# ruizhecao96/CMGAN

Measured on NVIDIA H100. Metric: utterances/sec (2 s @16 kHz) generator fwd+bwd, higher is better.
Workload: dtype tf32

## Files before the change

### cmgan_b200/csrc/gemm_tc.cu

```cuda
#include <cuda.h>

#include "common.cuh"
#include "../../include/cmgan_b200.h"
#include "gemm_device.cuh"
#include "tc_ptx.cuh"

namespace {
using namespace cmgan_gemm;
using namespace cmgan_tc;

constexpr int BM = 64;
constexpr int KC = 32;
constexpr int A_STAGE_BYTES = BM * KC * 4;
constexpr int NPROD = 128;
constexpr int NTHREADS = 256;
constexpr int SLAB = 64;
constexpr int STG_LD = SLAB + 4;
constexpr int STG_BYTES = 4 * 16 * STG_LD * 4;
constexpr int SMEM_LIMIT = 227 * 1024;
constexpr int SMEM_LIMIT2 = 112 * 1024;
constexpr int RESIDENT_MAX = 96 * 1024;

__global__ void pack_b_kernel(const float* __restrict__ B, long sb_tap, long sb_k, long sb_n, int Cin, int ntaps, int N, int BN,
                              float* __restrict__ out) {
    long total = (long)ntaps * (Cin / KC) * BN * KC;
    long i = (long)blockIdx.x * blockDim.x + threadIdx.x;
    if (i >= total) return;
    int kk = (int)(i % KC); long t = i / KC; int n = (int)(t % BN); long chunk = t / BN;
    int cpt = Cin / KC;
    int tap = (int)(chunk / cpt), kc = (int)(chunk % cpt);
    float v = 0.f;
    if (n < N) v = to_tf32(__ldg(B + (long)tap * sb_tap + (long)(kc * KC + kk) * sb_k + (long)n * sb_n));
    int c = kk >> 2, j = kk & 3;
    out[(chunk * BN + n) * KC + ((c ^ (n & 7)) << 2) + j] = v;
}

__global__ void pack_all_kernel(const CmganPackDesc* __restrict__ descs) {
    const CmganPackDesc d = descs[blockIdx.y];
    const int Cin = (int)d.Cin, N = (int)d.N;
    const long total = d.ntaps * (Cin / KC) * (long)N * KC;
    for (long i = (long)blockIdx.x * blockDim.x + threadIdx.x; i < total; i += (long)gridDim.x * blockDim.x) {
        int kk = (int)(i % KC); long t = i / KC; int n = (int)(t % N); long chunk = t / N;
        int cpt = Cin / KC;
        int tap = (int)(chunk / cpt), kc = (int)(chunk % cpt);
        float v = to_tf32(__ldg(d.src + (long)tap * d.sb_tap + (long)(kc * KC + kk) * d.sb_k + (long)n * d.sb_n));
        int c = kk >> 2, j = kk & 3;
        d.dst[(chunk * N + n) * KC + ((c ^ (n & 7)) << 2) + j] = v;
    }
}

struct TcCfg { int BN, stages, resident, ntiles, tma, nfx, nty, W, H; };
constexpr int PW = 8, PH = 8;

template <bool ASYNC_A, int NBMAX, int EPI, bool PATCH>
__global__ void __launch_bounds__(NTHREADS, NBMAX == 4 ? 2 : 1) gemm_rows_tc_kernel(const __grid_constant__ CmganGemmArgs g, const float* __restrict__ Bp,
                                                                                  const TcCfg cfg, const __grid_constant__ CUtensorMap tmA) {
    extern __shared__ uint8_t smem_raw[];
    const uint32_t base = (smem_u32(smem_raw) + 1023u) & ~1023u;
    uint8_t* base_ptr = smem_raw + (base - smem_u32(smem_raw));
    const int BN = cfg.BN, stages = cfg.stages;
    const int b_tile_bytes = BN * KC * 4;
    const int cpt = g.Cin / KC;
    const int nchunks = cpt * g.ntaps;
    const uint32_t sA = base;
    const uint32_t sB = sA + stages * A_STAGE_BYTES;
    const uint32_t b_region = (uint32_t)(cfg.resident ? nchunks : stages) * b_tile_bytes;
    const uint32_t sStg = sB + b_region;
    const uint32_t bars = sStg + STG_BYTES;
    auto full_bar = [&](int s) { return bars + 8u * s; };
    auto empty_bar = [&](int s) { return bars + 8u * (stages + s); };
    const uint32_t bready_bar = bars + 8u * (2 * stages);

    const int tid = threadIdx.x, warp = tid >> 5, lane = tid & 31;
    const int ntiles = cfg.ntiles;
    const int my_tiles = (ntiles - (int)blockIdx.x + (int)gridDim.x - 1) / (int)gridDim.x;

    if (tid == 0) {
        for (int s = 0; s < stages; ++s) { mbar_init(full_bar(s), cfg.tma ? 1 : NPROD + (cfg.resident ? 0 : 1)); mbar_init(empty_bar(s), 4); }
        mbar_init(bready_bar, 1);
        fence_barrier_init();
    }
    __syncthreads();

    if (warp < 4) {
        const int c = tid & 7;
        const int rr = tid >> 3;
        uint32_t dst_off[4];
#pragma unroll
        for (int i = 0; i < 4; ++i) { const int r = rr + 16 * i; dst_off[i] = r * 128 + ((c ^ (r & 7)) << 4); }
        const long total = (long)my_tiles * nchunks;
        if (tid == 0 && cfg.resident) {
            mbar_arrive_expect_tx(bready_bar, (uint32_t)(nchunks * b_tile_bytes));
            for (int ch = 0; ch < nchunks; ++ch)
                bulk_g2s(sB + ch * b_tile_bytes, Bp + (long)ch * BN * KC, (uint32_t)b_tile_bytes, bready_bar);
        }
#define B_STAGE(q, s)                                                                                                    \
        if (tid == 0 && !cfg.resident) {                                                                                 \
            if (!cfg.tma) mbar_arrive_expect_tx(full_bar(s), (uint32_t)b_tile_bytes);                                    \
            bulk_g2s(sB + (s) * b_tile_bytes, Bp + (long)((q) % nchunks) * BN * KC, (uint32_t)b_tile_bytes, full_bar(s)); \
        }

        if (ASYNC_A && cfg.tma) {
            if (tid == 0) {
                for (long q = 0; q < total; ++q) {
                    const int lt = (int)(q / nchunks), ch = (int)(q - (long)lt * nchunks);
                    const int s = (int)(q % stages);
                    const uint32_t par = (uint32_t)((q / stages) & 1);
                    mbar_wait(empty_bar(s), par ^ 1u);
                    mbar_arrive_expect_tx(full_bar(s), (uint32_t)(A_STAGE_BYTES + (cfg.resident ? 0 : b_tile_bytes)));
                    B_STAGE(q, s)
                    const int tile = blockIdx.x + lt * gridDim.x;
                    if (!PATCH) {
                        tma_load_2d(sA + s * A_STAGE_BYTES, &tmA, ch * KC, tile * BM, full_bar(s));
                    } else {
                        const int fx = tile % cfg.nfx, ty = (tile / cfg.nfx) % cfg.nty, bimg = tile / (cfg.nfx * cfg.nty);
                        const int tap = ch / cpt, kc = ch - tap * cpt;
                        tma_load_4d(sA + s * A_STAGE_BYTES, &tmA, kc * KC, fx * PW + g.dx[tap], ty * PH + g.dy[tap], bimg, full_bar(s));
                    }
                }
            }
            __syncwarp();
        } else if (ASYNC_A) {
            const int LAG = stages >= 3 ? 2 : 1;
            long rowoff[4];
            RowInfo ri[4];
            int cur_tile = -1, cur_tap = -1;
            for (long q = 0; q < total + LAG; ++q) {
                if (q < total) {
                    const int lt = (int)(q / nchunks), ch = (int)(q - (long)lt * nchunks);
                    const int s = (int)(q % stages);
                    const uint32_t par = (uint32_t)((q / stages) & 1);
                    const int tap = ch / cpt, k0 = (ch - tap * cpt) * KC + c * 4;
                    if (lt != cur_tile) {
                        cur_tile = lt; cur_tap = -1;
                        const int m0 = (blockIdx.x + lt * gridDim.x) * BM;
#pragma unroll
                        for (int i = 0; i < 4; ++i) ri[i] = decode_row(g, m0 + rr + 16 * i);
                    }
                    if (tap != cur_tap) {
                        cur_tap = tap;
#pragma unroll
                        for (int i = 0; i < 4; ++i) {
                            long r = in_row_of(g, ri[i], tap);
                            rowoff[i] = r < 0 ? -1 : g.tap_off[tap] + r * g.lda;
                        }
                    }
                    mbar_wait(empty_bar(s), par ^ 1u);
                    B_STAGE(q, s)
                    const uint32_t sbase = sA + s * A_STAGE_BYTES;
#pragma unroll
                    for (int i = 0; i < 4; ++i) {
                        const bool ok = rowoff[i] >= 0;
                        cp_async16(sbase + dst_off[i], g.A + (ok ? rowoff[i] + k0 : 0), ok ? 16u : 0u);
                    }
                }
                cp_async_commit();
                const long done = q - LAG;
                if (done >= 0) {
                    if (LAG == 2) cp_async_wait<2>(); else cp_async_wait<1>();
                    fence_proxy_async();
                    mbar_arrive(full_bar((int)(done % stages)));
                }
            }
        } else {
            float mean[4], rstd[4];
            RowInfo ri[4];
            int cur_tile = -1;
            for (long q = 0; q < total; ++q) {
                const int lt = (int)(q / nchunks), ch = (int)(q - (long)lt * nchunks);
                const int s = (int)(q % stages);
                const uint32_t par = (uint32_t)((q / stages) & 1);
                const int tap = ch / cpt, k0 = (ch - tap * cpt) * KC + c * 4;
                if (lt != cur_tile) {
                    cur_tile = lt;
                    const int m0 = (blockIdx.x + lt * gridDim.x) * BM;
#pragma unroll
                    for (int i = 0; i < 4; ++i) {
                        ri[i] = decode_row(g, m0 + rr + 16 * i);
                        mean[i] = 0.f; rstd[i] = 1.f;
                        if (g.pro == CMGAN_PRO_LN) {
                            long r = in_row_of(g, ri[i], 0);
                            if (r >= 0) { float2 st = __ldg(reinterpret_cast<const float2*>(g.p0) + r); mean[i] = st.x; rstd[i] = st.y; }
                        }
                    }
                }
                ChunkParams cp;
                load_chunk_params(g, k0, cp);
                float4 v[4];
                long rows[4];
#pragma unroll
                for (int i = 0; i < 4; ++i) {
                    rows[i] = in_row_of(g, ri[i], tap);
                    v[i] = rows[i] >= 0 ? __ldg(reinterpret_cast<const float4*>(g.A + g.tap_off[tap] + rows[i] * g.lda + k0)) : make_float4(0.f, 0.f, 0.f, 0.f);
                }
#pragma unroll
                for (int i = 0; i < 4; ++i)
                    if (rows[i] >= 0) v[i] = transform4(g, v[i], rows[i], k0, mean[i], rstd[i], cp);
                mbar_wait(empty_bar(s), par ^ 1u);
                B_STAGE(q, s)
                const uint32_t sbase = sA + s * A_STAGE_BYTES;
#pragma unroll
                for (int i = 0; i < 4; ++i)
                    asm volatile("st.shared.v4.f32 [%0], {%1, %2, %3, %4};" ::"r"(sbase + dst_off[i]), "f"(to_tf32(v[i].x)), "f"(to_tf32(v[i].y)),
                                 "f"(to_tf32(v[i].z)), "f"(to_tf32(v[i].w)) : "memory");
                fence_proxy_async();
                mbar_arrive(full_bar(s));
            }
        }
#undef B_STAGE
    } else {
        const int cw = warp - 4;
        const int nb = BN / 16;
        float acc[NBMAX][8];
#pragma unroll
        for (int j = 0; j < NBMAX; ++j)
#pragma unroll
            for (int i = 0; i < 8; ++i) acc[j][i] = 0.f;
        float* stg = reinterpret_cast<float*>(base_ptr + (sStg - base)) + cw * 16 * STG_LD;
        const int col4 = (lane & 15) * 4;
        const int rsub = lane >> 4;
        const int fg = lane >> 2, ft = lane & 3;
        constexpr bool DROPS = EPI == CMGAN_EPI_DROP_RES || EPI == CMGAN_EPI_DSWISH_DROP || EPI == CMGAN_EPI_SWISH_DUAL;
        const uint32_t seed32 = DROPS ? cmgan_seed32(eff_seed(g)) : 0u;
        const uint32_t thr16 = g.drop_thr >> 16;
        const bool drop_on = DROPS && g.drop_thr != 0u;
        constexpr bool patch = PATCH;
        const float inv_keep = g.inv_keep, alpha = g.alpha;
        const float* xbase = nullptr;
        long ldx = 0;
        if (EPI == CMGAN_EPI_DROP_RES) { xbase = g.R; ldx = g.ldr; }
        else if (EPI == CMGAN_EPI_DSWISH_DROP || EPI == CMGAN_EPI_DBNSWISH) { xbase = g.aux; ldx = g.ldaux; }
        else if (EPI == CMGAN_EPI_ACC) { xbase = g.C; ldx = g.ldc; }
        if (cfg.resident) mbar_wait(bready_bar, 0);
        long q = 0;
        for (int lt = 0; lt < my_tiles; ++lt) {
            for (int ch = 0; ch < nchunks; ++ch, ++q) {
                const int s = (int)(q % stages);
                const uint32_t par = (uint32_t)((q / stages) & 1);
                mbar_wait(full_bar(s), par);
                const uint64_t adesc = gmma_desc_sw128(sA + s * A_STAGE_BYTES);
                const uint64_t bdesc = gmma_desc_sw128(sB + (cfg.resident ? ch : s) * b_tile_bytes);
                wgmma_fence();
                mma_chunk_n<NBMAX>(nb, acc, adesc, bdesc, ch == 0);
                wgmma_commit();
                wgmma_wait<0>();
                __syncwarp();
                if (lane == 0) mbar_arrive(empty_bar(s));
            }
            const int tile = blockIdx.x + lt * gridDim.x;
            long mfirst;
            int hi_rows, vhi, vlo;
            if (patch) {
                const int fx = tile % cfg.nfx, ty = (tile / cfg.nfx) % cfg.nty, bimg = tile / (cfg.nfx * cfg.nty);
                const int y0 = ty * PH + cw * 2, x0 = fx * PW;
                mfirst = ((long)bimg * cfg.H + y0) * cfg.W + x0 + rsub;
                hi_rows = cfg.W; vhi = cfg.H - y0; vlo = cfg.W - x0;
            } else {
                const int mrow0 = tile * BM + cw * 16;
                mfirst = (long)mrow0 + rsub;
                hi_rows = 8; vhi = 2; vlo = g.M - mrow0;
            }
            auto row_ok = [&](int ps) { return patch ? ((ps >> 2) < vhi && 2 * (ps & 3) + rsub < vlo) : (2 * ps + rsub < vlo); };
            auto row_delta = [&](int ps) { return (long)(ps >> 2) * hi_rows + 2 * (ps & 3); };
            const bool any_row = row_ok(0);
#pragma unroll
            for (int sl = 0; sl < NBMAX / 4; ++sl) {
                const int n0 = sl * SLAB;
                if (n0 >= BN) break;
                const int ncols = min(SLAB, BN - n0);
#pragma unroll
                for (int jj = 0; jj < 4; ++jj) {
                    if (16 * jj >= ncols) break;
                    const float* d = acc[4 * sl + jj];
#pragma unroll
                    for (int i = 0; i < 2; ++i) {
                        const int col = 16 * jj + 8 * i + 2 * ft;
                        *reinterpret_cast<float2*>(stg + fg * STG_LD + col) = make_float2(d[4 * i], d[4 * i + 1]);
                        *reinterpret_cast<float2*>(stg + (fg + 8) * STG_LD + col) = make_float2(d[4 * i + 2], d[4 * i + 3]);
                    }
                }
                __syncwarp();
                if (col4 < ncols && any_row) {
                    const int n = n0 + col4;
                    float4 bias4 = make_float4(0.f, 0.f, 0.f, 0.f), e0v = bias4, e1v = bias4;
                    if (g.bias) bias4 = __ldg(reinterpret_cast<const float4*>(g.bias + n));
                    if (EPI == CMGAN_EPI_DBNSWISH) { e0v = __ldg(reinterpret_cast<const float4*>(g.e0 + n)); e1v = __ldg(reinterpret_cast<const float4*>(g.e1 + n)); }
                    float* cptr = g.C ? g.C + mfirst * g.ldc + n : nullptr;
                    float* c2ptr = EPI == CMGAN_EPI_SWISH_DUAL ? g.C2 + mfirst * g.ldc2 + n : nullptr;
                    const float* xp = xbase ? xbase + mfirst * ldx + n : nullptr;
                    const float* sptr = stg + rsub * STG_LD + col4;
                    const long ldc = g.ldc, ldc2 = g.ldc2;
                    const uint32_t pair = (uint32_t)(((unsigned long long)mfirst * (unsigned long long)g.N + (unsigned long long)n) >> 1);
                    const uint32_t phalf = (uint32_t)g.N >> 1;
#pragma unroll
                    for (int b4 = 0; b4 < 2; ++b4) {
                        float4 ex[4];
#pragma unroll
                        for (int u = 0; u < 4; ++u)
                            ex[u] = (xp && row_ok(b4 * 4 + u)) ? __ldg(reinterpret_cast<const float4*>(xp + row_delta(b4 * 4 + u) * ldx))
                                                                : make_float4(0.f, 0.f, 0.f, 0.f);
#pragma unroll
                        for (int u = 0; u < 4; ++u) {
                            const int ps = b4 * 4 + u;
                            if (!row_ok(ps)) continue;
                            const long rd = row_delta(ps);
                            const float4 a = *reinterpret_cast<const float4*>(sptr + ps * 2 * STG_LD);
                            float v[4] = {a.x + bias4.x, a.y + bias4.y, a.z + bias4.z, a.w + bias4.w};
                            float ds[4] = {1.f, 1.f, 1.f, 1.f};
                            if (DROPS && drop_on) {
                                const uint32_t pr = pair + (uint32_t)rd * phalf;
                                const uint32_t h0 = cmgan_mix32((pr * 0x9E3779B1u) ^ seed32), h1 = cmgan_mix32(((pr + 1u) * 0x9E3779B1u) ^ seed32);
                                ds[0] = (h0 & 0xFFFFu) >= thr16 ? inv_keep : 0.f; ds[1] = (h0 >> 16) >= thr16 ? inv_keep : 0.f;
                                ds[2] = (h1 & 0xFFFFu) >= thr16 ? inv_keep : 0.f; ds[3] = (h1 >> 16) >= thr16 ? inv_keep : 0.f;
                            }
                            const float x[4] = {ex[u].x, ex[u].y, ex[u].z, ex[u].w};
                            if (EPI == CMGAN_EPI_SWISH_DUAL) {
                                if (cptr) *reinterpret_cast<float4*>(cptr + rd * ldc) = make_float4(v[0], v[1], v[2], v[3]);
#pragma unroll
                                for (int j = 0; j < 4; ++j) v[j] = to_tf32(swishf_(v[j]) * ds[j]);
                                *reinterpret_cast<float4*>(c2ptr + rd * ldc2) = make_float4(v[0], v[1], v[2], v[3]);
                                continue;
                            }
                            if (EPI == CMGAN_EPI_DROP_RES) {
#pragma unroll
                                for (int j = 0; j < 4; ++j) v[j] = alpha * v[j] * ds[j] + (xbase ? x[j] : 0.f);
                            } else if (EPI == CMGAN_EPI_DSWISH_DROP) {
#pragma unroll
                                for (int j = 0; j < 4; ++j) v[j] = to_tf32(v[j] * dswishf_(x[j]) * ds[j]);
                            } else if (EPI == CMGAN_EPI_DBNSWISH) {
                                const float sa[4] = {e0v.x, e0v.y, e0v.z, e0v.w}, sb[4] = {e1v.x, e1v.y, e1v.z, e1v.w};
#pragma unroll
                                for (int j = 0; j < 4; ++j) v[j] = v[j] * dswishf_(fmaf(x[j], sa[j], sb[j]));
                            } else if (EPI == CMGAN_EPI_ACC) {
#pragma unroll
                                for (int j = 0; j < 4; ++j) v[j] = alpha * v[j] + x[j];
                            }
                            *reinterpret_cast<float4*>(cptr + rd * ldc) = make_float4(v[0], v[1], v[2], v[3]);
                        }
                    }
                }
                __syncwarp();
            }
        }
    }
}

int tc_supported(const CmganGemmArgs* a) {
    if (a->N % 16 || a->N < 16 || a->N > 256) return 0;
    if (a->Cin % KC) return 0;
    if (a->lda % 4 || ((uintptr_t)a->A & 15)) return 0;
    if (a->C && (a->ldc % 4 || ((uintptr_t)a->C & 15))) return 0;
    if (a->epi == CMGAN_EPI_SWISH_DUAL && (a->ldc2 % 4 || ((uintptr_t)a->C2 & 15))) return 0;
    if (a->bias && ((uintptr_t)a->bias & 15)) return 0;
    for (int t = 0; t < a->ntaps; ++t)
        if (a->tap_off[t] % 4) return 0;
    if (!a->ws || a->ws_floats < (long long)a->N * a->Cin * a->ntaps) return 0;
    if ((uintptr_t)a->ws & 127) return 0;
    if (a->pro == CMGAN_PRO_LN && (((uintptr_t)a->p1 & 15) || ((uintptr_t)a->p2 & 15) || a->ntaps != 1)) return 0;
    if (a->pro == CMGAN_PRO_BN_SWISH && (((uintptr_t)a->p0 & 15) || ((uintptr_t)a->p1 & 15))) return 0;
    if (a->pro == CMGAN_PRO_IN_PRELU && (((uintptr_t)a->p0 & 15) || ((uintptr_t)a->p1 & 15) || ((uintptr_t)a->p2 & 15) || a->pstride % 4)) return 0;
    return 1;
}

int g_num_sms = 0;

using PFN_encodeTiled = CUresult (*)(CUtensorMap*, CUtensorMapDataType, cuuint32_t, void*, const cuuint64_t*, const cuuint64_t*, const cuuint32_t*,
                                      const cuuint32_t*, CUtensorMapInterleave, CUtensorMapSwizzle, CUtensorMapL2promotion, CUtensorMapFloatOOBfill);
PFN_encodeTiled get_encoder() {
    static PFN_encodeTiled encode = nullptr;
    static bool tried = false;
    if (!tried) {
        tried = true;
        void* fn = nullptr;
        cudaDriverEntryPointQueryResult qres;
        if (cudaGetDriverEntryPoint("cuTensorMapEncodeTiled", &fn, cudaEnableDefault, &qres) == cudaSuccess && qres == cudaDriverEntryPointSuccess)
            encode = reinterpret_cast<PFN_encodeTiled>(fn);
    }
    return encode;
}

template <bool ASYNC_A, int NBMAX, int EPI, bool PATCH = false>
int launch_variant(const CmganGemmArgs& a, const TcCfg& cfg, int grid, size_t smem, cudaStream_t st, const CUtensorMap& tm) {
    static bool attr_set = false;
    if (!attr_set) {
        cudaError_t e = cudaFuncSetAttribute(gemm_rows_tc_kernel<ASYNC_A, NBMAX, EPI, PATCH>, cudaFuncAttributeMaxDynamicSharedMemorySize, SMEM_LIMIT);
        if (e != cudaSuccess) { cmgan_set_error("gemm_rows_tc: cudaFuncSetAttribute: %s", cudaGetErrorString(e)); return -1; }
        attr_set = true;
    }
    gemm_rows_tc_kernel<ASYNC_A, NBMAX, EPI, PATCH><<<grid, NTHREADS, smem, st>>>(a, a.ws, cfg, tm);
    return 0;
}

}

int cmgan_gemm_rows_tc_launch(const CmganGemmArgs* a, cudaStream_t st) {
    if (!tc_supported(a)) return 1;
    TcCfg cfg;
    cfg.BN = a->N;
    const int b_tile = cfg.BN * KC * 4;
    const int nchunks = (a->Cin / KC) * a->ntaps;
    cfg.resident = (long)nchunks * b_tile <= RESIDENT_MAX ? 1 : 0;
    const int resident_bytes = cfg.resident ? nchunks * b_tile : 0;
    const int per_stage = A_STAGE_BYTES + (cfg.resident ? 0 : b_tile);
    const int fixed = 1024  + STG_BYTES + 256  + resident_bytes;
    const int ctas = (a->pro == CMGAN_PRO_NONE && cfg.BN <= 64 && fixed + 3 * per_stage <= SMEM_LIMIT2) ? 2 : 1;
    const bool narrow = ctas == 2;
    cfg.stages = ((ctas == 2 ? SMEM_LIMIT2 : SMEM_LIMIT) - fixed) / per_stage;
    if (cfg.stages > 8) cfg.stages = 8;
    if (cfg.stages < 2) return 1;
    cfg.ntiles = cdiv(a->M, BM);
    const size_t smem = (size_t)fixed + (size_t)cfg.stages * per_stage;
    if (g_num_sms == 0) {
        int dev = 0;
        cudaGetDevice(&dev);
        cudaDeviceGetAttribute(&g_num_sms, cudaDevAttrMultiProcessorCount, dev);
    }
    alignas(64) CUtensorMap tm;
    memset(&tm, 0, sizeof(tm));
    cfg.tma = 0;
    cfg.nfx = cfg.nty = 1; cfg.W = cfg.H = 0;
    if (a->pro == CMGAN_PRO_NONE && !a->conv && a->ntaps == 1 && a->lda % 4 == 0) {
        PFN_encodeTiled encode = get_encoder();
        if (encode) {
            const cuuint64_t gdim[2] = {(cuuint64_t)a->Cin, (cuuint64_t)a->M};
            const cuuint64_t gstride[1] = {(cuuint64_t)a->lda * sizeof(float)};
            const cuuint32_t box[2] = {(cuuint32_t)KC, (cuuint32_t)BM};
            const cuuint32_t estr[2] = {1, 1};
            CUresult r = encode(&tm, CU_TENSOR_MAP_DATA_TYPE_FLOAT32, 2, const_cast<float*>(a->A + a->tap_off[0]), gdim, gstride, box, estr,
                                CU_TENSOR_MAP_INTERLEAVE_NONE, CU_TENSOR_MAP_SWIZZLE_128B, CU_TENSOR_MAP_L2_PROMOTION_L2_256B,
                                CU_TENSOR_MAP_FLOAT_OOB_FILL_NONE);
            if (r == CUDA_SUCCESS) cfg.tma = 1;
        }
    }
    bool same_off = true;
    for (int t = 1; t < a->ntaps; ++t) same_off = same_off && a->tap_off[t] == a->tap_off[0];
    if (a->pro == CMGAN_PRO_NONE && (a->epi == CMGAN_EPI_NONE || a->epi == CMGAN_EPI_ACC) && a->conv && a->mul_y == 1 && a->mul_x == 1 && a->div_y == 1 && a->div_x == 1 && a->OH == a->IH &&
        a->OW == a->IW && same_off && a->M % ((long long)a->OH * a->OW) == 0) {
        PFN_encodeTiled encode = get_encoder();
        if (encode) {
            const long long Bn = a->M / ((long long)a->OH * a->OW);
            const cuuint64_t gdim[4] = {(cuuint64_t)a->Cin, (cuuint64_t)a->IW, (cuuint64_t)a->IH, (cuuint64_t)Bn};
            const cuuint64_t gstride[3] = {(cuuint64_t)a->lda * sizeof(float), (cuuint64_t)a->IW * a->lda * sizeof(float),
                                           (cuuint64_t)a->IH * a->IW * a->lda * sizeof(float)};
            const cuuint32_t box[4] = {(cuuint32_t)KC, (cuuint32_t)PW, (cuuint32_t)PH, 1};
            const cuuint32_t estr[4] = {1, 1, 1, 1};
            CUresult r = encode(&tm, CU_TENSOR_MAP_DATA_TYPE_FLOAT32, 4, const_cast<float*>(a->A + a->tap_off[0]), gdim, gstride, box, estr,
                                CU_TENSOR_MAP_INTERLEAVE_NONE, CU_TENSOR_MAP_SWIZZLE_128B, CU_TENSOR_MAP_L2_PROMOTION_L2_256B,
                                CU_TENSOR_MAP_FLOAT_OOB_FILL_NONE);
            const long long nfx = cdiv(a->OW, PW), nty = cdiv(a->OH, PH);
            if (r == CUDA_SUCCESS && Bn * nfx * nty < (1ll << 30)) {
                cfg.tma = 2; cfg.nfx = (int)nfx; cfg.nty = (int)nty; cfg.W = a->OW; cfg.H = a->OH;
                cfg.ntiles = (int)(Bn * nfx * nty);
            }
        }
    }
    if (!a->b_packed) {
        long total = (long)nchunks * cfg.BN * KC;
        pack_b_kernel<<<cdiv(total, 256), 256, 0, st>>>(a->B, a->sb_tap, a->sb_k, a->sb_n, a->Cin, a->ntaps, a->N, cfg.BN, a->ws);
        if (cmgan_check_launch("pack_b_kernel")) return -1;
    }
    const int grid = cfg.ntiles < ctas * g_num_sms ? cfg.ntiles : ctas * g_num_sms;
    const int variant = a->pro != CMGAN_PRO_NONE ? 0 : (narrow ? 1 : 2);
    int rc = -2;
#define CMGAN_TC_LAUNCH(E)                                                                                            \
    case E:                                                                                                           \
        rc = variant == 0   ? launch_variant<false, 16, E>(*a, cfg, grid, smem, st, tm)                               \
             : variant == 1 ? launch_variant<true, 4, E>(*a, cfg, grid, smem, st, tm)                                 \
                            : launch_variant<true, 16, E>(*a, cfg, grid, smem, st, tm);                               \
        break;
    if (cfg.tma == 2) {
        if (a->epi == CMGAN_EPI_NONE)
            rc = narrow ? launch_variant<true, 4, CMGAN_EPI_NONE, true>(*a, cfg, grid, smem, st, tm)
                        : launch_variant<true, 16, CMGAN_EPI_NONE, true>(*a, cfg, grid, smem, st, tm);
        else
            rc = narrow ? launch_variant<true, 4, CMGAN_EPI_ACC, true>(*a, cfg, grid, smem, st, tm)
                        : launch_variant<true, 16, CMGAN_EPI_ACC, true>(*a, cfg, grid, smem, st, tm);
    } else
    switch (a->epi) {
        CMGAN_TC_LAUNCH(CMGAN_EPI_NONE)
        CMGAN_TC_LAUNCH(CMGAN_EPI_DROP_RES)
        CMGAN_TC_LAUNCH(CMGAN_EPI_DSWISH_DROP)
        CMGAN_TC_LAUNCH(CMGAN_EPI_DBNSWISH)
        CMGAN_TC_LAUNCH(CMGAN_EPI_ACC)
        CMGAN_TC_LAUNCH(CMGAN_EPI_SWISH_DUAL)
        default: break;
    }
#undef CMGAN_TC_LAUNCH
    if (rc == -2) { cmgan_set_error("gemm_rows_tc: unknown epilogue %d", a->epi); return -1; }
    if (rc) return -1;
    return cmgan_check_launch("gemm_rows_tc_kernel");
}

CMGAN_API int cmgan_pack_weight(const float* src, float* dst, long long sb_tap, long long sb_k, long long sb_n, int Cin, int ntaps, int N, void* stream) {
    CMGAN_REQUIRE(src && dst && Cin > 0 && Cin % KC == 0 && ntaps >= 1 && N > 0, "cmgan_pack_weight: bad arguments (Cin must be a multiple of %d)", KC);
    const long total = (long)ntaps * Cin * N;
    pack_b_kernel<<<cdiv(total, 256), 256, 0, (cudaStream_t)stream>>>(src, sb_tap, sb_k, sb_n, Cin, ntaps, N, N, dst);
    return cmgan_check_launch("pack_b_kernel");
}

CMGAN_API int cmgan_pack_weights(const CmganPackDesc* descs, int n, void* stream) {
    CMGAN_REQUIRE(descs || n == 0, "cmgan_pack_weights: null table");
    if (n == 0) return 0;
    pack_all_kernel<<<dim3(48, n), 256, 0, (cudaStream_t)stream>>>(descs);
    return cmgan_check_launch("pack_all_kernel");
}
```

### cmgan_b200/csrc/tc_ptx.cuh

```cuda
#pragma once
#include "common.cuh"

namespace cmgan_tc {

__device__ __forceinline__ uint32_t smem_u32(const void* p) { return (uint32_t)__cvta_generic_to_shared(p); }

__device__ __forceinline__ void mbar_init(uint32_t bar, uint32_t count) {
    asm volatile("mbarrier.init.shared::cta.b64 [%0], %1;" ::"r"(bar), "r"(count) : "memory");
}
__device__ __forceinline__ void mbar_arrive(uint32_t bar) {
    asm volatile("mbarrier.arrive.shared::cta.b64 _, [%0];" ::"r"(bar) : "memory");
}
__device__ __forceinline__ void mbar_arrive_expect_tx(uint32_t bar, uint32_t bytes) {
    asm volatile("mbarrier.arrive.expect_tx.shared::cta.b64 _, [%0], %1;" ::"r"(bar), "r"(bytes) : "memory");
}
__device__ __forceinline__ void mbar_wait(uint32_t bar, uint32_t parity) {
    uint32_t done = 0;
    for (uint32_t spin = 0; !done; ++spin) {
        asm volatile("{\n\t.reg .pred p;\n\tmbarrier.try_wait.parity.shared::cta.b64 p, [%1], %2;\n\tselp.u32 %0, 1, 0, p;\n\t}"
                     : "=r"(done) : "r"(bar), "r"(parity) : "memory");
        if (spin > (1u << 28)) __trap();
    }
}
__device__ __forceinline__ bool mbar_test(uint32_t bar, uint32_t parity) {
    uint32_t done;
    asm volatile("{\n\t.reg .pred p;\n\tmbarrier.test_wait.parity.shared::cta.b64 p, [%1], %2;\n\tselp.u32 %0, 1, 0, p;\n\t}"
                 : "=r"(done) : "r"(bar), "r"(parity) : "memory");
    return done != 0;
}
__device__ __forceinline__ void fence_barrier_init() { asm volatile("fence.mbarrier_init.release.cluster;" ::: "memory"); }
__device__ __forceinline__ void fence_proxy_async() { asm volatile("fence.proxy.async.shared::cta;" ::: "memory"); }

__device__ __forceinline__ void bulk_g2s(uint32_t dst_smem, const void* src, uint32_t bytes, uint32_t bar) {
    asm volatile("cp.async.bulk.shared::cluster.global.mbarrier::complete_tx::bytes [%0], [%1], %2, [%3];"
                 ::"r"(dst_smem), "l"(src), "r"(bytes), "r"(bar) : "memory");
}
__device__ __forceinline__ void tma_load_2d(uint32_t dst_smem, const void* tmap, int c0, int c1, uint32_t bar) {
    asm volatile("cp.async.bulk.tensor.2d.shared::cluster.global.mbarrier::complete_tx::bytes [%0], [%1, {%2, %3}], [%4];"
                 ::"r"(dst_smem), "l"(tmap), "r"(c0), "r"(c1), "r"(bar) : "memory");
}
__device__ __forceinline__ void tma_load_3d(uint32_t dst_smem, const void* tmap, int c0, int c1, int c2, uint32_t bar) {
    asm volatile("cp.async.bulk.tensor.3d.shared::cluster.global.mbarrier::complete_tx::bytes [%0], [%1, {%2, %3, %4}], [%5];"
                 ::"r"(dst_smem), "l"(tmap), "r"(c0), "r"(c1), "r"(c2), "r"(bar) : "memory");
}
__device__ __forceinline__ void tma_load_4d(uint32_t dst_smem, const void* tmap, int c0, int c1, int c2, int c3, uint32_t bar) {
    asm volatile("cp.async.bulk.tensor.4d.shared::cluster.global.mbarrier::complete_tx::bytes [%0], [%1, {%2, %3, %4, %5}], [%6];"
                 ::"r"(dst_smem), "l"(tmap), "r"(c0), "r"(c1), "r"(c2), "r"(c3), "r"(bar) : "memory");
}
__device__ __forceinline__ void cp_async16(uint32_t dst_smem, const void* src, uint32_t src_bytes) {
    asm volatile("cp.async.cg.shared.global [%0], [%1], 16, %2;" ::"r"(dst_smem), "l"(src), "r"(src_bytes) : "memory");
}
__device__ __forceinline__ void cp_async8(uint32_t dst_smem, const void* src) {
    asm volatile("cp.async.ca.shared.global [%0], [%1], 8;" ::"r"(dst_smem), "l"(src) : "memory");
}
__device__ __forceinline__ void cp_async_commit() { asm volatile("cp.async.commit_group;" ::: "memory"); }
template <int N>
__device__ __forceinline__ void cp_async_wait() { asm volatile("cp.async.wait_group %0;" ::"n"(N) : "memory"); }

__device__ __forceinline__ float to_tf32(float x) {
    uint32_t r;
    asm("cvt.rna.tf32.f32 %0, %1;" : "=r"(r) : "f"(x));
    return __uint_as_float(r);
}

__device__ __forceinline__ uint64_t gmma_desc_sw128(uint32_t saddr) {
    uint64_t d = 0;
    d |= (uint64_t)((saddr & 0x3FFFF) >> 4);
    d |= (uint64_t)1 << 16;
    d |= (uint64_t)(1024 >> 4) << 32;
    d |= (uint64_t)1 << 62;
    return d;
}
__device__ __forceinline__ void wgmma_fence() { asm volatile("wgmma.fence.sync.aligned;" ::: "memory"); }
__device__ __forceinline__ void wgmma_commit() { asm volatile("wgmma.commit_group.sync.aligned;" ::: "memory"); }
template <int N>
__device__ __forceinline__ void wgmma_wait() { asm volatile("wgmma.wait_group.sync.aligned %0;" ::"n"(N) : "memory"); }
__device__ __forceinline__ void wgmma_m64n16k8_tf32(float d[8], uint64_t adesc, uint64_t bdesc, uint32_t accumulate) {
    asm volatile("{\n\t.reg .pred p;\n\tsetp.ne.b32 p, %10, 0;\n\t"
                 "wgmma.mma_async.sync.aligned.m64n16k8.f32.tf32.tf32 {%0, %1, %2, %3, %4, %5, %6, %7}, %8, %9, p, 1, 1;\n\t}"
                 : "+f"(d[0]), "+f"(d[1]), "+f"(d[2]), "+f"(d[3]), "+f"(d[4]), "+f"(d[5]), "+f"(d[6]), "+f"(d[7])
                 : "l"(adesc), "l"(bdesc), "r"(accumulate));
}
#define CMGAN_D8(b) "+f"(d[b][0]), "+f"(d[b][1]), "+f"(d[b][2]), "+f"(d[b][3]), "+f"(d[b][4]), "+f"(d[b][5]), "+f"(d[b][6]), "+f"(d[b][7])
__device__ __forceinline__ void wgmma_m64n64k8_tf32(float (&d)[4][8], uint64_t adesc, uint64_t bdesc, uint32_t accumulate) {
    asm volatile("{\n\t.reg .pred p;\n\tsetp.ne.b32 p, %34, 0;\n\t"
                 "wgmma.mma_async.sync.aligned.m64n64k8.f32.tf32.tf32 "
                 "{%0, %1, %2, %3, %4, %5, %6, %7, %8, %9, %10, %11, %12, %13, %14, %15, "
                 "%16, %17, %18, %19, %20, %21, %22, %23, %24, %25, %26, %27, %28, %29, %30, %31}, %32, %33, p, 1, 1;\n\t}"
                 : CMGAN_D8(0), CMGAN_D8(1), CMGAN_D8(2), CMGAN_D8(3)
                 : "l"(adesc), "l"(bdesc), "r"(accumulate));
}
__device__ __forceinline__ void wgmma_m64n64k8_tf32_rs(float (&d)[4][8], const uint32_t (&a)[4], uint64_t bdesc, uint32_t accumulate) {
    asm volatile("{\n\t.reg .pred p;\n\tsetp.ne.b32 p, %37, 0;\n\t"
                 "wgmma.mma_async.sync.aligned.m64n64k8.f32.tf32.tf32 "
                 "{%0, %1, %2, %3, %4, %5, %6, %7, %8, %9, %10, %11, %12, %13, %14, %15, "
                 "%16, %17, %18, %19, %20, %21, %22, %23, %24, %25, %26, %27, %28, %29, %30, %31}, {%32, %33, %34, %35}, %36, p, 1, 1;\n\t}"
                 : CMGAN_D8(0), CMGAN_D8(1), CMGAN_D8(2), CMGAN_D8(3)
                 : "r"(a[0]), "r"(a[1]), "r"(a[2]), "r"(a[3]), "l"(bdesc), "r"(accumulate));
}
#undef CMGAN_D8

template <int NB, int NBMAX>
__device__ __forceinline__ void mma_chunk(float (&acc)[NBMAX][8], uint64_t adesc, uint64_t bdesc, bool first) {
#pragma unroll
    for (int k = 0; k < 4; ++k)
#pragma unroll
        for (int j = 0; j < NB; ++j)
            wgmma_m64n16k8_tf32(acc[j], adesc + (uint64_t)(2 * k), bdesc + (uint64_t)(128 * j + 2 * k), (first && k == 0) ? 0u : 1u);
}
template <int NBMAX, int I = 1>
__device__ __forceinline__ void mma_chunk_n(int nb, float (&acc)[NBMAX][8], uint64_t adesc, uint64_t bdesc, bool first) {
    if constexpr (I <= NBMAX) {
        if (nb == I) mma_chunk<I, NBMAX>(acc, adesc, bdesc, first);
        else mma_chunk_n<NBMAX, I + 1>(nb, acc, adesc, bdesc, first);
    }
}

}
```

Before: 90.98.

## Use wide wgmma instructions and overlap MMA with the next chunk's barrier wait

Replaces the per-16-column m64n16k8 wgmma loop with a single wide m64nNk8 instruction (N = 64/128/192/256) per k-step, rounding the column-block count up to a multiple of four. The consumer loop now keeps one wgmma group in flight (wait<1>) and releases the previous stage's buffer late, so tensor-core work overlaps the next stage's barrier wait. It also reduces the producer lag for three-stage rings and adds a host-side early return for non-TMA configurations with fewer than three stages. Rounding up the width may compute wasted columns, and the new early return could reject configurations that used to run.

```diff
diff --git a/cmgan_b200/csrc/gemm_tc.cu b/cmgan_b200/csrc/gemm_tc.cu
--- a/cmgan_b200/csrc/gemm_tc.cu
+++ b/cmgan_b200/csrc/gemm_tc.cu
@@ -51,6 +51,38 @@
 
 struct TcCfg { int BN, stages, resident, ntiles, tma, nfx, nty, W, H; };
 constexpr int PW = 8, PH = 8;
+
+struct TileRing { uint32_t sA, sB, bars; int stages, b_tile_bytes, nchunks, resident, lane; };
+
+template <int NB, int NBMAX>
+__device__ __forceinline__ void tile_mma(float (&acc)[NBMAX][8], const TileRing& r, long& q) {
+    auto empty_bar = [&](long qq) { return r.bars + 8u * (r.stages + (int)(qq % r.stages)); };
+    for (int ch = 0; ch < r.nchunks; ++ch, ++q) {
+        const int s = (int)(q % r.stages);
+        const uint32_t par = (uint32_t)((q / r.stages) & 1);
+        mbar_wait(r.bars + 8u * s, par);
+        const uint64_t adesc = gmma_desc_sw128(r.sA + s * A_STAGE_BYTES);
+        const uint64_t bdesc = gmma_desc_sw128(r.sB + (r.resident ? ch : s) * r.b_tile_bytes);
+        wgmma_fence();
+        mma_chunk<NB, NBMAX>(acc, adesc, bdesc, ch == 0);
+        wgmma_commit();
+        wgmma_wait<1>();
+        if (ch > 0) {
+            __syncwarp();
+            if (r.lane == 0) mbar_arrive(empty_bar(q - 1));
+        }
+    }
+    wgmma_wait<0>();
+    __syncwarp();
+    if (r.lane == 0) mbar_arrive(empty_bar(q - 1));
+}
+template <int NBMAX, int I = 1>
+__device__ __forceinline__ void tile_mma_nw(int nw, float (&acc)[NBMAX][8], const TileRing& r, long& q) {
+    if constexpr (4 * I <= NBMAX) {
+        if (nw == I) tile_mma<4 * I, NBMAX>(acc, r, q);
+        else tile_mma_nw<NBMAX, I + 1>(nw, acc, r, q);
+    }
+}
 
 template <bool ASYNC_A, int NBMAX, int EPI, bool PATCH>
 __global__ void __launch_bounds__(NTHREADS, NBMAX == 4 ? 2 : 1) gemm_rows_tc_kernel(const __grid_constant__ CmganGemmArgs g, const float* __restrict__ Bp,
@@ -121,7 +153,7 @@
             }
             __syncwarp();
         } else if (ASYNC_A) {
-            const int LAG = stages >= 3 ? 2 : 1;
+            const int LAG = stages >= 4 ? 2 : 1;
             long rowoff[4];
             RowInfo ri[4];
             int cur_tile = -1, cur_tap = -1;
@@ -232,21 +264,10 @@
         else if (EPI == CMGAN_EPI_DSWISH_DROP || EPI == CMGAN_EPI_DBNSWISH) { xbase = g.aux; ldx = g.ldaux; }
         else if (EPI == CMGAN_EPI_ACC) { xbase = g.C; ldx = g.ldc; }
         if (cfg.resident) mbar_wait(bready_bar, 0);
+        const TileRing ring{sA, sB, bars, stages, b_tile_bytes, nchunks, cfg.resident, lane};
         long q = 0;
         for (int lt = 0; lt < my_tiles; ++lt) {
-            for (int ch = 0; ch < nchunks; ++ch, ++q) {
-                const int s = (int)(q % stages);
-                const uint32_t par = (uint32_t)((q / stages) & 1);
-                mbar_wait(full_bar(s), par);
-                const uint64_t adesc = gmma_desc_sw128(sA + s * A_STAGE_BYTES);
-                const uint64_t bdesc = gmma_desc_sw128(sB + (cfg.resident ? ch : s) * b_tile_bytes);
-                wgmma_fence();
-                mma_chunk_n<NBMAX>(nb, acc, adesc, bdesc, ch == 0);
-                wgmma_commit();
-                wgmma_wait<0>();
-                __syncwarp();
-                if (lane == 0) mbar_arrive(empty_bar(s));
-            }
+            tile_mma_nw<NBMAX>((nb + 3) / 4, acc, ring, q);
             const int tile = blockIdx.x + lt * gridDim.x;
             long mfirst;
             int hi_rows, vhi, vlo;
@@ -454,6 +475,7 @@
             }
         }
     }
+    if (a->pro == CMGAN_PRO_NONE && cfg.tma == 0 && cfg.stages < 3) return 1;
     if (!a->b_packed) {
         long total = (long)nchunks * cfg.BN * KC;
         pack_b_kernel<<<cdiv(total, 256), 256, 0, st>>>(a->B, a->sb_tap, a->sb_k, a->sb_n, a->Cin, a->ntaps, a->N, cfg.BN, a->ws);
diff --git a/cmgan_b200/csrc/tc_ptx.cuh b/cmgan_b200/csrc/tc_ptx.cuh
--- a/cmgan_b200/csrc/tc_ptx.cuh
+++ b/cmgan_b200/csrc/tc_ptx.cuh
@@ -100,20 +100,65 @@
 }
 #undef CMGAN_D8
 
+#define CMGAN_DJ(b) "+f"(d[b][0]), "+f"(d[b][1]), "+f"(d[b][2]), "+f"(d[b][3]), "+f"(d[b][4]), "+f"(d[b][5]), "+f"(d[b][6]), "+f"(d[b][7])
+template <int W, int NBMAX>
+__device__ __forceinline__ void wgmma_tf32_blocks(float (&d)[NBMAX][8], uint64_t adesc, uint64_t bdesc, uint32_t accumulate) {
+    static_assert(W <= NBMAX, "accumulator blocks out of range");
+    if constexpr (W == 4) {
+        wgmma_m64n64k8_tf32(*reinterpret_cast<float(*)[4][8]>(&d[0]), adesc, bdesc, accumulate);
+    } else if constexpr (W == 8) {
+        asm volatile("{\n\t.reg .pred p;\n\tsetp.ne.b32 p, %66, 0;\n\t"
+                     "wgmma.mma_async.sync.aligned.m64n128k8.f32.tf32.tf32 {"
+                     "%0, %1, %2, %3, %4, %5, %6, %7, %8, %9, %10, %11, %12, %13, %14, %15, "
+                     "%16, %17, %18, %19, %20, %21, %22, %23, %24, %25, %26, %27, %28, %29, %30, %31, "
+                     "%32, %33, %34, %35, %36, %37, %38, %39, %40, %41, %42, %43, %44, %45, %46, %47, "
+                     "%48, %49, %50, %51, %52, %53, %54, %55, %56, %57, %58, %59, %60, %61, %62, %63"
+                     "}, %64, %65, p, 1, 1;\n\t}"
+                     : CMGAN_DJ(0), CMGAN_DJ(1), CMGAN_DJ(2), CMGAN_DJ(3),
+                       CMGAN_DJ(4), CMGAN_DJ(5), CMGAN_DJ(6), CMGAN_DJ(7)
+                     : "l"(adesc), "l"(bdesc), "r"(accumulate));
+    } else if constexpr (W == 12) {
+        asm volatile("{\n\t.reg .pred p;\n\tsetp.ne.b32 p, %98, 0;\n\t"
+                     "wgmma.mma_async.sync.aligned.m64n192k8.f32.tf32.tf32 {"
+                     "%0, %1, %2, %3, %4, %5, %6, %7, %8, %9, %10, %11, %12, %13, %14, %15, "
+                     "%16, %17, %18, %19, %20, %21, %22, %23, %24, %25, %26, %27, %28, %29, %30, %31, "
+                     "%32, %33, %34, %35, %36, %37, %38, %39, %40, %41, %42, %43, %44, %45, %46, %47, "
+                     "%48, %49, %50, %51, %52, %53, %54, %55, %56, %57, %58, %59, %60, %61, %62, %63, "
+                     "%64, %65, %66, %67, %68, %69, %70, %71, %72, %73, %74, %75, %76, %77, %78, %79, "
+                     "%80, %81, %82, %83, %84, %85, %86, %87, %88, %89, %90, %91, %92, %93, %94, %95"
+                     "}, %96, %97, p, 1, 1;\n\t}"
+                     : CMGAN_DJ(0), CMGAN_DJ(1), CMGAN_DJ(2), CMGAN_DJ(3),
+                       CMGAN_DJ(4), CMGAN_DJ(5), CMGAN_DJ(6), CMGAN_DJ(7),
+                       CMGAN_DJ(8), CMGAN_DJ(9), CMGAN_DJ(10), CMGAN_DJ(11)
+                     : "l"(adesc), "l"(bdesc), "r"(accumulate));
+    } else if constexpr (W == 16) {
+        asm volatile("{\n\t.reg .pred p;\n\tsetp.ne.b32 p, %130, 0;\n\t"
+                     "wgmma.mma_async.sync.aligned.m64n256k8.f32.tf32.tf32 {"
+                     "%0, %1, %2, %3, %4, %5, %6, %7, %8, %9, %10, %11, %12, %13, %14, %15, "
+                     "%16, %17, %18, %19, %20, %21, %22, %23, %24, %25, %26, %27, %28, %29, %30, %31, "
+                     "%32, %33, %34, %35, %36, %37, %38, %39, %40, %41, %42, %43, %44, %45, %46, %47, "
+                     "%48, %49, %50, %51, %52, %53, %54, %55, %56, %57, %58, %59, %60, %61, %62, %63, "
+                     "%64, %65, %66, %67, %68, %69, %70, %71, %72, %73, %74, %75, %76, %77, %78, %79, "
+                     "%80, %81, %82, %83, %84, %85, %86, %87, %88, %89, %90, %91, %92, %93, %94, %95, "
+                     "%96, %97, %98, %99, %100, %101, %102, %103, %104, %105, %106, %107, %108, %109, %110, %111, "
+                     "%112, %113, %114, %115, %116, %117, %118, %119, %120, %121, %122, %123, %124, %125, %126, %127"
+                     "}, %128, %129, p, 1, 1;\n\t}"
+                     : CMGAN_DJ(0), CMGAN_DJ(1), CMGAN_DJ(2), CMGAN_DJ(3),
+                       CMGAN_DJ(4), CMGAN_DJ(5), CMGAN_DJ(6), CMGAN_DJ(7),
+                       CMGAN_DJ(8), CMGAN_DJ(9), CMGAN_DJ(10), CMGAN_DJ(11),
+                       CMGAN_DJ(12), CMGAN_DJ(13), CMGAN_DJ(14), CMGAN_DJ(15)
+                     : "l"(adesc), "l"(bdesc), "r"(accumulate));
+    } else {
+        static_assert(W == 4, "no wgmma wrapper for this width");
+    }
+}
+#undef CMGAN_DJ
+
 template <int NB, int NBMAX>
 __device__ __forceinline__ void mma_chunk(float (&acc)[NBMAX][8], uint64_t adesc, uint64_t bdesc, bool first) {
 #pragma unroll
     for (int k = 0; k < 4; ++k)
-#pragma unroll
-        for (int j = 0; j < NB; ++j)
-            wgmma_m64n16k8_tf32(acc[j], adesc + (uint64_t)(2 * k), bdesc + (uint64_t)(128 * j + 2 * k), (first && k == 0) ? 0u : 1u);
-}
-template <int NBMAX, int I = 1>
-__device__ __forceinline__ void mma_chunk_n(int nb, float (&acc)[NBMAX][8], uint64_t adesc, uint64_t bdesc, bool first) {
-    if constexpr (I <= NBMAX) {
-        if (nb == I) mma_chunk<I, NBMAX>(acc, adesc, bdesc, first);
-        else mma_chunk_n<NBMAX, I + 1>(nb, acc, adesc, bdesc, first);
-    }
+        wgmma_tf32_blocks<NB, NBMAX>(acc, adesc + (uint64_t)(2 * k), bdesc + (uint64_t)(2 * k), (first && k == 0) ? 0u : 1u);
 }
 
 }
```

After: 94.87, median of 6. +4.3%, better.
